# sbelharbi/sr-caco-2

Measured on AMD Instinct MI355X. Metric: train patches/sec, SwinIR x8 64->512 1ch, higher is better.
Workload: dtype f32 (fp16x2 split-MFMA, f32 accumulate)

## Files before the change

sr-caco-2_amd/csrc/gemm_tnb.hip:

```cpp
#include <stdlib.h>
#include "common.h"
#include "kernels.h"

typedef __bf16 bf16x8 __attribute__((ext_vector_type(8)));
typedef __bf16 bf16x2 __attribute__((ext_vector_type(2)));
typedef float f32x2 __attribute__((ext_vector_type(2)));
typedef unsigned u32x4 __attribute__((ext_vector_type(4)));

namespace {

constexpr int TKB = 32;

__device__ const float k_tnb_zero_row[256] = {0.f};

__device__ __forceinline__ f32x16 mfma_bf(u32x4 a, u32x4 b, f32x16 c) {
  return __builtin_amdgcn_mfma_f32_32x32x16_bf16(__builtin_bit_cast(bf16x8, a),
                                                 __builtin_bit_cast(bf16x8, b), c, 0, 0, 0);
}

typedef _Float16 f16x8 __attribute__((ext_vector_type(8)));
typedef _Float16 tn_f16x2 __attribute__((ext_vector_type(2)));
__device__ __forceinline__ f32x16 mfma_h(u32x4 a, u32x4 b, f32x16 c) {
  return __builtin_amdgcn_mfma_f32_32x32x16_f16(__builtin_bit_cast(f16x8, a), __builtin_bit_cast(f16x8, b), c, 0, 0, 0);
}
__device__ __forceinline__ void split2_pair(float x0, float x1, unsigned& h, unsigned& l) {
  const tn_f16x2 hv = __builtin_convertvector(f32x2{x0, x1}, tn_f16x2);
  const float r0 = x0 - (float)hv.x, r1 = x1 - (float)hv.y;
  const tn_f16x2 lv = __builtin_convertvector(f32x2{r0, r1}, tn_f16x2);
  h = __builtin_bit_cast(unsigned, hv);
  l = __builtin_bit_cast(unsigned, lv);
}

template <int W>
__device__ __forceinline__ int unit_slot(int col, int u) {
  if (W == 2) {
    const int x = col ^ (col >> 4);
    return 4 * ((col & ~3) | (x & 3)) + (u ^ ((x >> 2) & 3));
  }
  return 4 * col + (u ^ ((col >> 2) & 3));
}

typedef float tnb_f32x3 __attribute__((ext_vector_type(3)));
typedef tnb_f32x3 __attribute__((aligned(4))) tnb_f32x3_u;
template <int W> struct ColVec;
template <> struct ColVec<1> {
  typedef float T;
  static __device__ __forceinline__ T ldg(const float* p) { return ldg_f(p); }
  static __device__ __forceinline__ T ldg(const float* base, unsigned off) {
    return *(sr_gptr_f)((const char*)base + off);
  }
  static __device__ __forceinline__ float at(T v, int) { return v; }
};
template <> struct ColVec<2> {
  typedef sr_f32x2 T;
  static __device__ __forceinline__ T ldg(const float* p) { return *(sr_gptr_f2)p; }
  static __device__ __forceinline__ T ldg(const float* base, unsigned off) {
    return *(sr_gptr_f2)((const char*)base + off);
  }
  static __device__ __forceinline__ float at(T v, int j) { return v[j]; }
};
template <> struct ColVec<3> {
  typedef tnb_f32x3 T;
  static __device__ __forceinline__ T ldg(const float* p) {
    return *(const __attribute__((address_space(1))) tnb_f32x3_u*)p;
  }
  static __device__ __forceinline__ T ldg(const float* base, unsigned off) {
    return *(const __attribute__((address_space(1))) tnb_f32x3_u*)((const char*)base + off);
  }
  static __device__ __forceinline__ float at(T v, int j) { return v[j]; }
};

template <int W>
__device__ __forceinline__ void tnb_body(const TnArgs& p, const int s, const int tile, const int tap,
                                         unsigned char* smem) {
  constexpr int BC = 64 * W;
  constexpr int PLANE = 2 * BC * 64;
  constexpr int BUF = 3 * PLANE;

  const int tid = threadIdx.x, lane = tid & 63;
  const int wave8 = __builtin_amdgcn_readfirstlane(tid >> 6);
  const bool producer = wave8 >= 4;
  const int wave = wave8 & 3;
  const int wi = wave >> 1, wj = wave & 1, r = lane & 31, h = lane >> 5;
  const int nbj = (p.NJ + p.j_tile - 1) / p.j_tile;
  const int bi = tile / nbj, bj = tile - bi * nbj;
  const int i0 = bi * p.i_tile, j0 = bj * p.j_tile;
  const int ivalid = min(p.i_tile, p.NI - i0), jvalid = min(p.j_tile, p.NJ - j0);
  const int m_begin = s * p.rows_per_slice;
  const int m_end = min(p.M, m_begin + p.rows_per_slice);
  const int dy = p.conv ? tap / 3 - 1 : 0, dx = p.conv ? tap % 3 - 1 : 0;
  const bool do_colsum = p.part_colsum && bj == 0 && tap == 0;

  struct Stage {
    typename ColVec<W>::T rv[2][8];
// ... 183 lines not shown
    load(m_begin + TKB, sg1);
    store(smem, sg0);
    load(m_begin + 2 * TKB, sg0);
    __syncthreads();
    for (int c = 0; c < nch; c += 2) {
      store(smem + BUF, sg1);
      load(m_begin + (c + 3) * TKB, sg1);
      __syncthreads();
      store(smem, sg0);
      load(m_begin + (c + 4) * TKB, sg0);
      __syncthreads();
    }
  } else {
    __syncthreads();
    for (int c = 0; c < nch; ++c) {
      const unsigned char* cur = smem + (c & 1) * BUF;
#pragma unroll
      for (int ks = 0; ks < 2; ++ks) {
        u32x4 fa[W][3];
#pragma unroll
        for (int i = 0; i < W; ++i)
#pragma unroll
          for (int pl = 0; pl < 3; ++pl) fa[i][pl] = *(const u32x4*)(cur + pl * PLANE + a_off[i][ks]);
#pragma unroll
        for (int j = 0; j < W; ++j) {
          u32x4 fb0 = *(const u32x4*)(cur + b_off[j][ks]);
          u32x4 fb1 = *(const u32x4*)(cur + PLANE + b_off[j][ks]);
          u32x4 fb2 = *(const u32x4*)(cur + 2 * PLANE + b_off[j][ks]);
#pragma unroll
          for (int i = 0; i < W; ++i) acc[i][j] = mfma_bf(fa[i][1], fb1, acc[i][j]);
#pragma unroll
          for (int i = 0; i < W; ++i) acc[i][j] = mfma_bf(fa[i][0], fb2, acc[i][j]);
#pragma unroll
          for (int i = 0; i < W; ++i) acc[i][j] = mfma_bf(fa[i][2], fb0, acc[i][j]);
#pragma unroll
          for (int i = 0; i < W; ++i) acc[i][j] = mfma_bf(fa[i][0], fb1, acc[i][j]);
#pragma unroll
          for (int i = 0; i < W; ++i) acc[i][j] = mfma_bf(fa[i][1], fb0, acc[i][j]);
#pragma unroll
          for (int i = 0; i < W; ++i) acc[i][j] = mfma_bf(fa[i][0], fb0, acc[i][j]);
        }
      }
      __syncthreads();
    }

  float* out = p.part + ((long)(s * (p.conv ? 9 : 1) + tap) * p.NI) * p.NJ;
#pragma unroll
  for (int i = 0; i < W; ++i)
#pragma unroll
    for (int j = 0; j < W; ++j) {
      const int col = (wj * W + j) * 32 + r;
      if (col >= jvalid) continue;
#pragma unroll
      for (int q = 0; q < 16; ++q) {
        const int row = (wi * W + i) * 32 + mfma_row(q, lane);
        if (row < ivalid) {
          const int io = i0 + row;
          out[(long)(p.ps ? (io % ps_f) * 4 + io / ps_f : io) * p.NJ + j0 + col] = acc[i][j][q];
        }
      }
    }
  }

  if (do_colsum) {
    float* red = (float*)smem;
    if (producer && !isB) {
#pragma unroll
      for (int j = 0; j < W; ++j) red[hh * BC + W * lane + j] = cs[j];
    }
    __syncthreads();
    if (tid < ivalid) {
      const int io = i0 + tid;
      p.part_colsum[(long)s * p.NI + (p.ps ? (io % ps_f) * 4 + io / ps_f : io)] = red[tid] + red[BC + tid];
    }
  }
}

template <int W, int BM = -1, bool AR = false, bool NR = false, bool CONV = false>
__device__ __forceinline__ void tnb_body_h(const TnArgs& p, const int s, const int tile, unsigned char* smem, const int tap = 0) {
  const int bmode = BM >= 0 ? BM : p.b_mode;
  const bool arow = BM >= 0 ? AR : (p.a_rowscale != nullptr);
  constexpr int BC = 64 * W, HC = 32 * W;
  constexpr int PLANE = 2 * BC * 64;
  constexpr int BUF = 3 * PLANE;
  constexpr int CTRL = 2 * PLANE;
  constexpr int SINV = 2 * PLANE + 4096;

  const int tid = threadIdx.x, lane = tid & 63;
  const int wave8 = __builtin_amdgcn_readfirstlane(tid >> 6);
  const bool producer = wave8 >= 4;
  const int wave = wave8 & 3;
  const int wi = wave >> 1, wj = wave & 1, r = lane & 31, h = lane >> 5;
  const int nbj = (p.NJ + p.j_tile - 1) / p.j_tile;
  const int bi = tile / nbj, bj = tile - bi * nbj;
  const int i0 = bi * p.i_tile, j0 = bj * p.j_tile;
  const int ivalid = min(p.i_tile, p.NI - i0), jvalid = min(p.j_tile, p.NJ - j0);
  const int m_begin = s * p.rows_per_slice;
  const int m_end = min(p.M, m_begin + p.rows_per_slice);
  const bool do_colsum = p.part_colsum && bj == 0 && tap == 0;
  const int cdy = CONV ? tap / 3 - 1 : 0, cdx = CONV ? tap % 3 - 1 : 0;

  struct Stage {
    typename ColVec<W>::T rv[2][8];
    float scale;
    float2 stats;
    int trow;
  };
  Stage sg0, sg1;
  const bool isB = wave & 1;
  const int ch = wave >> 1;
  const int lt = lane & 31, th = lane >> 5;
  const int opvalid = isB ? jvalid : ivalid;
  const int gcol = HC * ch + W * lt;
  const int colq = max(min(gcol, opvalid - W), 0);
  const int dsh = gcol - colq;
  const bool ragged = NR ? false : opvalid % W != 0;
  const float* const opP = isB ? p.B + j0 : p.A + i0;
  const long opLd = isB ? p.ldb : p.lda;
  const unsigned colb = (unsigned)((16L * th * opLd + colq) * 4);
  float cs[W], sc[W];
#pragma unroll
  for (int j = 0; j < W; ++j) { cs[j] = 0.f; sc[j] = 0x1p126f; }

  auto bcast_i = [&](int v, int k) __attribute__((always_inline)) -> int {
    const int lo = __builtin_amdgcn_readlane(v, k), hi = __builtin_amdgcn_readlane(v, 16 + k);
    return th ? hi : lo;
  };
  const unsigned ld4 = (unsigned)opLd * 4u, colb0 = (unsigned)colq * 4u;
  auto load_c = [&](int mc, Stage& sg) __attribute__((always_inline)) {
    const int gm = mc + (lane & 31);
    bool ok = gm < m_end;
    int srow = gm;
    const int x = gm % p.Wd, tq = gm / p.Wd;
    const int y = tq % p.H, bq = tq / p.H;
    const int yy = y + (isB ? cdy : 0), xx = x + (isB ? cdx : 0);
    ok = ok && yy >= 0 && yy < p.H && xx >= 0 && xx < p.Wd;
    srow = (bq * p.H + yy) * p.Wd + xx;
    sg.trow = ok ? srow : -1;
#pragma unroll
    for (int t = 0; t < 16; ++t) {
      const int row = max(bcast_i(sg.trow, t), 0);
      sg.rv[t >> 3][t & 7] = ColVec<W>::ldg(opP, (unsigned)row * ld4 + colb0);
    }
  };
  auto load = [&](int mc, Stage& sg) __attribute__((always_inline)) {
    const int tokl = mc + (lane & 31);
    const bool interior = mc + TKB <= m_end;
    const bool tin = interior || tokl < m_end;
    if (!isB) sg.scale = ldg_f((arow && tin) ? p.a_rowscale + tokl / p.a_rowscale_rows : k_sr_neutral + 1);
    else sg.stats = ldg_f2((bmode == 1 && tin) ? p.ln_stats + 2 * (long)tokl : k_sr_neutral);
    const float* q = opP + (long)mc * opLd;
    if (interior) {
#pragma unroll
      for (int t = 0; t < 16; ++t) {
        sg.rv[t >> 3][t & 7] = ColVec<W>::ldg(q, colb);
        q += opLd;
      }
    } else {
#pragma unroll
      for (int t = 0; t < 16; ++t) {
        const bool ok = mc + 16 * th + t < m_end;
        sg.rv[t >> 3][t & 7] = ColVec<W>::ldg(ok ? (const float*)((const char*)q + colb) : k_tnb_zero_row);
        q += opLd;
      }
    }
  };
  auto load_i = [&](int mc, Stage& sg) __attribute__((always_inline)) {
// ... 175 lines not shown
      store(smem, sg0);
      load(m_begin + 2 * TKB, sg0);
      __syncthreads();
    }
    for (; c < nch; c += 2) {
      store(smem + BUF, sg1);
      load(m_begin + (c + 3) * TKB, sg1);
      __syncthreads();
      store(smem, sg0);
      load(m_begin + (c + 4) * TKB, sg0);
      __syncthreads();
    }
    if (th == 0) {
#pragma unroll
      for (int j = 0; j < W; ++j) ((float*)(smem + SINV))[(isB ? BC : 0) + gcol + j] = 1.0f / sc[j];
    }
    __syncthreads();
  } else {
    __syncthreads();
    for (int c = 0; c < nch; ++c) {
      const unsigned char* cur = smem + (c & 1) * BUF;
      const float* ctrl = (const float*)(cur + CTRL);
      const u32x4 fl = *(const u32x4*)(ctrl + 2 * BC);
      if (__builtin_amdgcn_readfirstlane(fl.x | fl.y | fl.z | fl.w)) {
        float fb[W];
#pragma unroll
        for (int j = 0; j < W; ++j) fb[j] = ctrl[BC + (wj * W + j) * 32 + r];
#pragma unroll
        for (int i = 0; i < W; ++i)
#pragma unroll
          for (int q = 0; q < 16; ++q) {
            const float fa = ctrl[(wi * W + i) * 32 + mfma_row(q, lane)];
#pragma unroll
            for (int j = 0; j < W; ++j) acc[i][j][q] *= fa * fb[j];
          }
      }
#pragma unroll
      for (int ks = 0; ks < 2; ++ks) {
        u32x4 fa[W][2];
#pragma unroll
        for (int i = 0; i < W; ++i)
#pragma unroll
          for (int pl = 0; pl < 2; ++pl) fa[i][pl] = *(const u32x4*)(cur + pl * PLANE + a_off[i][ks]);
#pragma unroll
        for (int j = 0; j < W; ++j) {
          const u32x4 bh = *(const u32x4*)(cur + b_off[j][ks]);
          const u32x4 bl = *(const u32x4*)(cur + PLANE + b_off[j][ks]);
#pragma unroll
          for (int i = 0; i < W; ++i) acc[i][j] = mfma_h(fa[i][1], bh, acc[i][j]);
#pragma unroll
          for (int i = 0; i < W; ++i) acc[i][j] = mfma_h(fa[i][0], bl, acc[i][j]);
#pragma unroll
          for (int i = 0; i < W; ++i) acc[i][j] = mfma_h(fa[i][0], bh, acc[i][j]);
        }
      }
      __syncthreads();
    }
    __syncthreads();
    const float* sinv = (const float*)(smem + SINV);
    float* out = p.part + ((long)(s * (CONV ? 9 : 1) + tap) * p.NI) * p.NJ;
#pragma unroll
    for (int i = 0; i < W; ++i)
#pragma unroll
      for (int j = 0; j < W; ++j) {
        const int col = (wj * W + j) * 32 + r;
        if (col >= jvalid) continue;
        const float ib = sinv[BC + col];
#pragma unroll
        for (int q = 0; q < 16; ++q) {
          const int row = (wi * W + i) * 32 + mfma_row(q, lane);
          if (row < ivalid) out[(long)(i0 + row) * p.NJ + j0 + col] = acc[i][j][q] * (sinv[row] * ib);
        }
      }
  }

  if (do_colsum) {
    float* red = (float*)smem;
    if (producer && !isB) {
#pragma unroll
      for (int j = 0; j < W; ++j) red[th * BC + gcol + j] = cs[j];
    }
    __syncthreads();
    if (tid < ivalid) p.part_colsum[(long)s * p.NI + i0 + tid] = red[tid] + red[BC + tid];
  }
}

constexpr int TK9 = 16;
__device__ __forceinline__ int unit_slot9(int col, int u) { return 2 * col + (u ^ ((col >> 3) & 1)); }
constexpr int T9_OPS = 6;
constexpr int T9_PLANE = T9_OPS * 64 * 32;
constexpr int T9_CTRL = 2 * T9_PLANE;
constexpr int T9_BUF = 2 * T9_PLANE + 2048;
constexpr int T9_SINV = 2 * T9_BUF;
constexpr int T9_LDS = 2 * T9_BUF + 2048;
constexpr int T9_THREADS = 14 * 64;

template <int H2, int DBG = 0>
__device__ __forceinline__ void tnb9_consume(const TnArgs& p, const int s, const int i0, const int j0, const int nch,
                                             unsigned char* smem, const int wi, const int wj, const int lane) {
  constexpr int NU = H2 ? 4 : 5;
  constexpr int DY0 = H2 ? 1 : 0;
  const int r = lane & 31, h = lane >> 5;
  f32x16 acc[NU];
#pragma unroll
  for (int u = 0; u < NU; ++u)
#pragma unroll
    for (int q = 0; q < 16; ++q) acc[u][q] = 0.f;
  int a_off[3], b_off[2];
#pragma unroll
  for (int d = 0; d < 3; ++d) a_off[d] = unit_slot9(d * 64 + wi * 32 + r, h) * 16;
#pragma unroll
  for (int d = 0; d < 2; ++d) b_off[d] = unit_slot9((3 + DY0 + d) * 64 + wj * 32 + r, h) * 16;
  __syncthreads();
  long long ts0 = 0, ts1 = 0;
  if (DBG == 3) ts0 = (long long)wall_clock64();
  for (int c = 0; c < nch; ++c) {
    const unsigned char* cur = smem + (c & 1) * T9_BUF;
    const float* ctrl = (const float*)(cur + T9_CTRL);
    const u32x4 f0 = *(const u32x4*)(ctrl + T9_OPS * 64);
    const sr_u32x2 f1 = *(const sr_u32x2*)(ctrl + T9_OPS * 64 + 4);
    if (__builtin_amdgcn_readfirstlane(f0.x | f0.y | f0.z | f0.w | f1.x | f1.y)) {
      const unsigned fl[6] = {f0.x, f0.y, f0.z, f0.w, f1.x, f1.y};
#pragma unroll
      for (int u = 0; u < NU; ++u) {
        constexpr int T0 = 5 * H2;
        const int t = T0 + u, dyi = t / 3, dxi = t - 3 * dyi;
        if (fl[dxi] | fl[3 + dyi]) {
          const float fb = fl[3 + dyi] ? ctrl[(3 + dyi) * 64 + wj * 32 + r] : 1.f;
#pragma unroll
          for (int q = 0; q < 16; ++q) acc[u][q] *= (fl[dxi] ? ctrl[dxi * 64 + wi * 32 + mfma_row(q, lane)] : 1.f) * fb;
        }
      }
    }
    u32x4 ah[3], al[3], bh[2], bl[2];
    const u32x4 dummy = u32x4{(unsigned)lane, 0x3c003c00u, 0x3c003c00u, (unsigned)c};
#pragma unroll
    for (int d = 0; d < 2; ++d) {
      bh[d] = (DBG >= 6) ? dummy : *(const u32x4*)(cur + b_off[d]);
      bl[d] = (DBG >= 6) ? dummy : *(const u32x4*)(cur + T9_PLANE + b_off[d]);
    }
#pragma unroll
    for (int dx = 0; dx < 3; ++dx) {
      ah[dx] = (DBG >= 6) ? dummy : *(const u32x4*)(cur + a_off[dx]);
      al[dx] = (DBG >= 6) ? dummy : *(const u32x4*)(cur + T9_PLANE + a_off[dx]);
    }
    if (DBG != 1) {
#pragma unroll
      for (int term = 0; term < 3; ++term) {
#pragma unroll
        for (int u = 0; u < NU; ++u) {
          const int t = 5 * H2 + u, dyi = t / 3, dxi = t - 3 * dyi;
          if (DBG == 10) {
            acc[u] = mfma_bf(term == 0 ? al[dxi] : ah[dxi], term == 1 ? bl[dyi - DY0] : bh[dyi - DY0], acc[u]);
          } else if (term == 0) acc[u] = mfma_h(al[dxi], bh[dyi - DY0], acc[u]);
          else if (term == 1) acc[u] = mfma_h(ah[dxi], bl[dyi - DY0], acc[u]);
          else acc[u] = mfma_h(ah[dxi], bh[dyi - DY0], acc[u]);
        }
      }
    }
    if (DBG != 8 && DBG != 10) __syncthreads();
  }
  if (DBG == 3) ts1 = (long long)wall_clock64();
  if (DBG != 9) __syncthreads();
  const float* sinv = (const float*)(smem + T9_SINV);
  const int col = wj * 32 + r;
  const int ps_f = p.NI >> 2;
// ... 402 lines not shown
      __syncthreads();
    }
    if (half == 0) ((float*)(smem + S9_SINV))[(isB ? 64 : 0) + lane] = 1.0f / sc;
    mxs[sw * 64 + lane] = mxrun;
    if (colsum && !isB) ((float*)(smem + S9_CS))[half * 64 + lane] = cs;
    __syncthreads();
    if (!pass) {
      aux[64 + sw * 64 + lane] = mxrun;
      const float mcol = fmaxf(mxrun, mxs[(sw ^ 1) * 64 + lane]);
      const float top = mcol * sc;
      const bool over = __any(top > 60000.f), under = __any(mcol > 0.f && top < 0.125f);
      if ((over || under) && lane == 0) *(volatile int*)(smem + S9_RETRY) = 1;
      if (lane == 0) ((int*)aux)[1 + sw] = (over ? 1 : 0) | (under ? 2 : 0);
    }
    __syncthreads();
    if (!pass && sw == 0 && lane == 0) *(int*)aux = *(volatile const int*)(smem + S9_RETRY);
  }
  if (colsum) {
    __syncthreads();
    if (sw == 0 && lane_ok) {
      const float* c2 = (const float*)(smem + S9_CS);
      const int io = i0 + lane;
      p.part_colsum[(long)s * p.NI + (p.ps ? (io % ps_f) * 4 + io / ps_f : io)] = c2[lane] + c2[64 + lane];
    }
  }
}

template <int DBG = 0, int PASS = 0>
__global__ void __launch_bounds__(S9_THREADS) k_tnb9s(TnArgs p, int tiles, int xcd) {
  extern __shared__ __attribute__((aligned(16))) unsigned char smem[];
  const int L = xcd ? sr_xcd_block(blockIdx.x, gridDim.x) : (int)blockIdx.x;
  tnb_body9s<DBG>(p, L / tiles, L % tiles, tiles, PASS, smem);
}

template <int W>
__global__ void __launch_bounds__(512, 1) k_tnb(TnArgs p, int tiles, int xcd) {
  extern __shared__ __attribute__((aligned(16))) unsigned char smem[];
  if (!p.conv) { tnb_body<W>(p, blockIdx.x, blockIdx.y, 0, smem); return; }
  const int L = xcd ? sr_xcd_block(blockIdx.x, gridDim.x) : (int)blockIdx.x;
  const int tap = L % 9, t2 = L / 9;
  tnb_body<W>(p, t2 / tiles, t2 % tiles, tap, smem);
}

template <int W>
__global__ void __launch_bounds__(512, 1) k_tnb_hc(TnArgs p, int tiles, int xcd) {
  extern __shared__ __attribute__((aligned(16))) unsigned char smem[];
  const int L = xcd ? sr_xcd_block(blockIdx.x, gridDim.x) : (int)blockIdx.x;
  const int tap = L % 9, t2 = L / 9;
  const bool even = p.NI % W == 0 && p.NJ % W == 0 && p.i_tile % W == 0 && p.j_tile % W == 0;
  if (even) tnb_body_h<W, 0, false, true, true>(p, t2 / tiles, t2 % tiles, smem, tap);
  else tnb_body_h<W, 0, false, false, true>(p, t2 / tiles, t2 % tiles, smem, tap);
}

constexpr int TNB_GROUP_MAX = 24;
struct TnbGroup {
  TnArgs p[TNB_GROUP_MAX];
  int tile_start[TNB_GROUP_MAX + 1];
  int n, S, xcd;
};
__device__ __forceinline__ void tnb_group_block(const TnbGroup& g, int& slice, int& t) {
  const int tiles = g.tile_start[g.n];
  if (g.xcd) {
    const int L = sr_xcd_block(blockIdx.x, gridDim.x);
    t = L % tiles;
    slice = L / tiles;
  } else {
    slice = blockIdx.x % g.S;
    t = blockIdx.x / g.S;
  }
}
template <int W>
__global__ void __launch_bounds__(512, 1) k_tnb_grouped(TnbGroup g) {
  extern __shared__ __attribute__((aligned(16))) unsigned char smem[];
  int slice, t;
  tnb_group_block(g, slice, t);
  TnArgs p = g.p[0];
  int t0 = 0;
#pragma unroll
  for (int i = 1; i < TNB_GROUP_MAX; ++i)
    if (i < g.n && t >= g.tile_start[i]) { p = g.p[i]; t0 = g.tile_start[i]; }
  tnb_body<W>(p, slice, t - t0, 0, smem);
}

template <int W>
__global__ void __launch_bounds__(512, 1) k_tnb_grouped_h(TnbGroup g) {
  extern __shared__ __attribute__((aligned(16))) unsigned char smem[];
  int slice, t;
  tnb_group_block(g, slice, t);
  TnArgs p = g.p[0];
  int t0 = 0;
#pragma unroll
  for (int i = 1; i < TNB_GROUP_MAX; ++i)
    if (i < g.n && t >= g.tile_start[i]) { p = g.p[i]; t0 = g.tile_start[i]; }
  const bool even = p.NI % W == 0 && p.NJ % W == 0 && p.i_tile % W == 0 && p.j_tile % W == 0;
  if (even && p.b_mode == 1 && !p.a_rowscale) tnb_body_h<W, 1, false, true>(p, slice, t - t0, smem);
  else if (even && p.b_mode == 0 && p.a_rowscale) tnb_body_h<W, 0, true, true>(p, slice, t - t0, smem);
  else if (even && p.b_mode == 2 && p.a_rowscale) tnb_body_h<W, 2, true, true>(p, slice, t - t0, smem);
  else tnb_body_h<W>(p, slice, t - t0, smem);
}

constexpr int TNB_BATCH_MAX = 40;
struct TnbConvBatch {
  TnArgs base;
  const float* A[TNB_BATCH_MAX];
  const float* B[TNB_BATCH_MAX];
  long part_stride, colsum_stride;
  int n, tiles, xcd;
};
template <int W>
__global__ void __launch_bounds__(512, 1) k_tnb_conv_batched(TnbConvBatch g) {
  extern __shared__ __attribute__((aligned(16))) unsigned char smem[];
  const int L = g.xcd ? sr_xcd_block(blockIdx.x, gridDim.x) : (int)blockIdx.x;
  const int tap = L % 9;
  int rr = L / 9;
  const int tile = rr % g.tiles; rr /= g.tiles;
  const int sl = rr % g.base.S, k = rr / g.base.S;
  TnArgs p = g.base;
  p.A = g.A[k];
  p.B = g.B[k];
  p.part = g.base.part + (long)k * g.part_stride;
  p.part_colsum = g.base.part_colsum ? g.base.part_colsum + (long)k * g.colsum_stride : nullptr;
  tnb_body<W>(p, sl, tile, tap, smem);
}

__global__ void __launch_bounds__(T9_THREADS) k_tnb9_conv_batched(TnbConvBatch g) {
  extern __shared__ __attribute__((aligned(16))) unsigned char smem[];
  const int L = g.xcd ? sr_xcd_block(blockIdx.x, gridDim.x) : (int)blockIdx.x;
  int rr = L;
  const int tile = rr % g.tiles; rr /= g.tiles;
  const int sl = rr % g.base.S, k = rr / g.base.S;
  TnArgs p = g.base;
  p.A = g.A[k];
  p.B = g.B[k];
  p.part = g.base.part + (long)k * g.part_stride;
  p.part_colsum = g.base.part_colsum ? g.base.part_colsum + (long)k * g.colsum_stride : nullptr;
  tnb_body9<0>(p, sl, tile, smem);
}

template <int PASS>
__global__ void __launch_bounds__(S9_THREADS) k_tnb9s_conv_batched(TnbConvBatch g) {
  extern __shared__ __attribute__((aligned(16))) unsigned char smem[];
  auto one = [&](int L) __attribute__((always_inline)) {
    int rr = L;
    const int tile = rr % g.tiles; rr /= g.tiles;
    const int sl = rr % g.base.S, k = rr / g.base.S;
    TnArgs p = g.base;
    p.A = g.A[k];
    p.B = g.B[k];
    p.part = g.base.part + (long)k * g.part_stride;
    p.part_colsum = g.base.part_colsum ? g.base.part_colsum + (long)k * g.colsum_stride : nullptr;
    p.aux = g.base.aux + (long)k * g.base.S * g.tiles * S9_AUX;
    tnb_body9s<0>(p, sl, tile, g.tiles, PASS, smem);
  };
  one(g.xcd ? sr_xcd_block(blockIdx.x, gridDim.x) : (int)blockIdx.x);
}

int pick_tile(int n, int* w) {
  if (n % 180 == 0) { *w = 3; return 180; }
  if (n <= 64) { *w = 1; return 64; }
  if (n <= 128 || n % 128 == 0) { *w = 2; return 128; }
  *w = 3; return 192;
}

int pick_w(int NI, int NJ, int* tile) {
  int wi, wj;
  const int ti = pick_tile(NI, &wi), tj = pick_tile(NJ, &wj);
  const int w = wi < wj ? wi : wj;
  *tile = wi == wj ? ti : (w == 3 ? 192 : 64 * w);
  if (wi == wj && ti != tj) *tile = 64 * w;
  return w;
}

enum TnbForm {
  TNB_PLAIN,
  TNB_HC,
  TNB_NINE,
  TNB_STRIP9,
};

TnbForm tnb_form(int conv, int NI, int NJ, const TnArgs* p = nullptr) {
#ifdef SR_TN_T9S_OFF
  constexpr int strip = 0;
#else
  static const int strip = [] { const char* e = sr_getenv("SRHIP_TN_T9S"); return !(e && e[0] == '0'); }();
#endif
  static const int ragged = [] { const char* e = sr_getenv("SRHIP_TN_T9S_RAGGED"); return e ? atoi(e) : 1; }();
  static const int f16c3 = [] { const char* e = sr_getenv("SRHIP_TN_F16X2_CONV3"); return e ? atoi(e) : 1; }();
  if (!conv || (p && (p->a_rowscale || p->b_mode != 0))) return TNB_PLAIN;
  int tile;
  const int w = pick_w(NI, NJ, &tile);
  const bool nine = w == 1 && NI % 64 == 0 && NJ % 64 == 0;
  if (strip && (nine || (ragged && NI >= 64 && NJ >= 64)) &&
      (!p || (p->Wd % 64 == 0 && p->S >= p->Wd / 64 && (!p->ps || NI % 64 == 0) &&
              (long)p->batch * p->H * (p->Wd / 64) >= 4L * p->S)))
    return TNB_STRIP9;
  if (nine) return TNB_NINE;
  if (w >= 2 && f16c3 &&
      (!p || (!p->ps && (long)p->M * p->lda < (1L << 30) && (long)p->batch * p->H * p->Wd * p->ldb < (1L << 30))))
    return TNB_HC;
  return TNB_PLAIN;
}
TnbForm tnb_form(const TnArgs& p) { return tnb_form(p.conv, p.NI, p.NJ, &p); }

long tnb_plan_blocks(int conv, int NI, int NJ, int* w, bool* nine) {
  int tile;
  *w = pick_w(NI, NJ, &tile);
  const TnbForm f = tnb_form(conv, NI, NJ);
  *nine = f == TNB_NINE || f == TNB_STRIP9;
  if (f == TNB_STRIP9) tile = 64;
  return (long)sr_cdiv(NI, tile) * sr_cdiv(NJ, tile) * (conv && !*nine ? 9 : 1);
}

template <typename K>
int reserve_lds(K kern, int bytes, const char* name) {
  hipError_t e = hipFuncSetAttribute((const void*)kern, hipFuncAttributeMaxDynamicSharedMemorySize, bytes);
  if (e != hipSuccess) return sr_fail(-5, "%s: cannot reserve %d B of LDS: %s", name, bytes, hipGetErrorString(e));
  return 0;
}

constexpr int lds_bytes(int w) { return 2 * 3 * 2 * 64 * w * 64; }
constexpr long TNB_W1_SLOTS = 3 * 256;

}

int sr_gemm_tnb_grouped(TnArgs* probs, int n, hipStream_t st) {
  SR_REQUIRE(n >= 1 && n <= TNB_GROUP_MAX, "gemm_tn_grouped_bx3: 1..%d problems (got %d)", TNB_GROUP_MAX, n);
  static_assert(sizeof(TnbGroup) <= 4096, "kernel arguments");
  TnbGroup g;
  memset(&g, 0, sizeof(g));
  g.n = n;
  int w = 1, tiles = 0;
  for (int k = 0; k < n; ++k) {
    TnArgs& p = probs[k];
    SR_REQUIRE(p.M == probs[0].M && p.S == probs[0].S && !p.conv,
               "gemm_tn_grouped_bx3: problems must share M and S");
    SR_REQUIRE(p.NI % 4 == 0 && p.NJ % 4 == 0 && p.lda % 4 == 0 && p.ldb % 4 == 0,
               "gemm_tn_grouped_bx3: NI, NJ, lda, ldb must be multiples of 4");
    int a, b;
    p.i_tile = pick_tile(p.NI, &a);
    p.j_tile = pick_tile(p.NJ, &b);
    if (a > w) w = a;
    if (b > w) w = b;
    const int rps = sr_cdiv(p.M, p.S);
    p.rows_per_slice = (rps + TKB - 1) / TKB * TKB;
    g.tile_start[k] = tiles;
    tiles += sr_cdiv(p.NI, p.i_tile) * sr_cdiv(p.NJ, p.j_tile);
    g.p[k] = p;
  }
  g.tile_start[n] = tiles;
  g.S = probs[0].S;
  static const int gxcd = [] { const char* e = sr_getenv("SRHIP_TN_GROUP_XCD"); return e ? atoi(e) : 1; }();
  g.xcd = gxcd;
  dim3 grid(probs[0].S * tiles, 1, 1);
  static bool attr[4] = {false, false, false, false};
#define SR_TNB_G(W_)                                                                      \
  if (w == W_) {                                                                          \
    if (!attr[W_]) {                                                                      \
      if (int rc = reserve_lds(k_tnb_grouped<W_>, lds_bytes(W_), "k_tnb_grouped")) return rc; \
      attr[W_] = true;                                                                    \
    }                                                                                     \
    hipLaunchKernelGGL((k_tnb_grouped<W_>), grid, dim3(512), lds_bytes(W_), st, g);       \
  }
  if (w == 3) {
    static bool attr_h = false;
    if (!attr_h) {
      if (int rc = reserve_lds(k_tnb_grouped_h<3>, lds_bytes(3), "k_tnb_grouped_h")) return rc;
      attr_h = true;
    }
    hipLaunchKernelGGL((k_tnb_grouped_h<3>), grid, dim3(512), lds_bytes(3), st, g);
  }
  SR_TNB_G(1) SR_TNB_G(2)
#undef SR_TNB_G
  SR_LAUNCH_CHECK("k_tnb_grouped");
  return 0;
}

int sr_gemm_tnb(TnArgs& p, hipStream_t st) {
  SR_REQUIRE(p.M > 0 && p.S > 0, "gemm_tn_bx3: empty problem");
  SR_REQUIRE(p.NI % 4 == 0 && p.NJ % 4 == 0 && p.lda % 4 == 0 && p.ldb % 4 == 0,
             "gemm_tn_bx3: NI, NJ, lda, ldb must be multiples of 4");
  int tile;
  const int w = pick_w(p.NI, p.NJ, &tile);
  p.i_tile = p.j_tile = tile;
  SR_REQUIRE(!p.ps || (p.conv && p.NI % 4 == 0 && (p.NI / 4) % w == 0 && p.NI % p.i_tile == 0),
             "conv3x3_wgrad + PixelShuffle(2): Cout/4 = %d must be a multiple of %d (columns per lane), Cout of the tile", p.NI / 4, w);
  const int rps = sr_cdiv(p.M, p.S);
  p.rows_per_slice = (rps + TKB - 1) / TKB * TKB;
  int tiles = sr_cdiv(p.NI, p.i_tile) * sr_cdiv(p.NJ, p.j_tile);
  dim3 grid(p.S, tiles, 1);
  if (p.conv) grid = dim3(p.S * tiles * 9, 1, 1);
  static const int xcd = [] { const char* e = sr_getenv("SRHIP_TN_XCD"); return !(e && e[0] == '0'); }();
  const TnbForm form = tnb_form(p);
  if (form == TNB_STRIP9) {
    p.i_tile = p.j_tile = 64;
    tiles = sr_cdiv(p.NI, 64) * sr_cdiv(p.NJ, 64);
    p.aux = p.part + (long)p.S * 9 * p.NI * p.NJ;
    static bool attr9s = false;
    if (!attr9s) {
      if (int rc = reserve_lds(k_tnb9s<0, 0>, S9_LDS, "k_tnb9s")) return rc;
      if (int rc = reserve_lds(k_tnb9s<0, 1>, S9_LDS, "k_tnb9s")) return rc;
      attr9s = true;
    }
#ifdef SRHIP_EXPERIMENTS
    {
      const char* e = sr_getenv("SRHIP_TN_DBG");
      const int dbg = e ? atoi(e) : 0;
#define SR_T9DBG(D_) if (dbg == D_) { reserve_lds(k_tnb9s<D_>, S9_LDS, "k_tnb9s"); hipLaunchKernelGGL(k_tnb9s<D_>, dim3(p.S * tiles), dim3(S9_THREADS), S9_LDS, st, p, tiles, xcd); return 0; }
      SR_T9DBG(1) SR_T9DBG(2) SR_T9DBG(6) SR_T9DBG(7)
#undef SR_T9DBG
    }
#endif
    hipLaunchKernelGGL((k_tnb9s<0, 0>), dim3(p.S * tiles), dim3(S9_THREADS), S9_LDS, st, p, tiles, xcd);
    hipLaunchKernelGGL((k_tnb9s<0, 1>), dim3(p.S * tiles), dim3(S9_THREADS), S9_LDS, st, p, tiles, xcd);
    SR_LAUNCH_CHECK("k_tnb9s");
    return 0;
  }
  if (form == TNB_NINE) {
    static bool attr9 = false;
    if (!attr9) {
      if (int rc = reserve_lds(k_tnb9<0>, T9_LDS, "k_tnb9")) return rc;
      attr9 = true;
    }
#ifdef SRHIP_EXPERIMENTS
    {
      const char* e = sr_getenv("SRHIP_TN_DBG");
      const int dbg = e ? atoi(e) : 0;
#define SR_T9DBG(D_) if (dbg == D_) { reserve_lds(k_tnb9<D_>, T9_LDS, "k_tnb9"); hipLaunchKernelGGL(k_tnb9<D_>, dim3(p.S * tiles), dim3(T9_THREADS), T9_LDS, st, p, tiles, xcd); return 0; }
      SR_T9DBG(1) SR_T9DBG(2) SR_T9DBG(6) SR_T9DBG(7) SR_T9DBG(3) SR_T9DBG(8) SR_T9DBG(9) SR_T9DBG(10) SR_T9DBG(4) SR_T9DBG(5)
#undef SR_T9DBG
    }
#endif
    hipLaunchKernelGGL(k_tnb9<0>, dim3(p.S * tiles), dim3(T9_THREADS), T9_LDS, st, p, tiles, xcd);
    SR_LAUNCH_CHECK("k_tnb9");
    return 0;
  }
  if (form == TNB_HC) {
    static bool attr_hc[4] = {false, false, false, false};
#define SR_TNB_HC(W_)                                                                       \
    if (w == W_) {                                                                          \
      if (!attr_hc[W_]) {                                                                   \
        if (int rc = reserve_lds(k_tnb_hc<W_>, lds_bytes(W_), "k_tnb_hc")) return rc;       \
        attr_hc[W_] = true;                                                                 \
      }                                                                                     \
      hipLaunchKernelGGL((k_tnb_hc<W_>), grid, dim3(512), lds_bytes(W_), st, p, tiles, xcd); \
    }
    SR_TNB_HC(2) SR_TNB_HC(3)
#undef SR_TNB_HC
    SR_LAUNCH_CHECK("k_tnb_hc");
    return 0;
  }
  static bool attr[4] = {false, false, false, false};
#define SR_TNB(W_)                                                                        \
  if (w == W_) {                                                                          \
    if (!attr[W_]) {                                                                      \
      if (int rc = reserve_lds(k_tnb<W_>, lds_bytes(W_), "k_tnb")) return rc;             \
      attr[W_] = true;                                                                    \
    }                                                                                     \
    hipLaunchKernelGGL((k_tnb<W_>), grid, dim3(512), lds_bytes(W_), st, p, tiles, xcd);   \
  }
  SR_TNB(1) SR_TNB(2) SR_TNB(3)
#undef SR_TNB
  SR_LAUNCH_CHECK("k_tnb");
  return 0;
}

int sr_conv_wgrad_batched_plan(int n, int M, int NI, int NJ, int* S, long* part_floats_per_item) {
  int w;
  bool t9;
  const long tiles = tnb_plan_blocks(1, NI, NJ, &w, &t9) * n;
  const long slots = w == 1 && !t9 ? TNB_W1_SLOTS : 256;
  long best = 1;
  double best_eff = 0.0;
  for (long s = 1; s <= 64; ++s) {
    if (s > 1 && M / s < 1024) break;
    const long blocks = tiles * s;
    const double eff = (double)blocks / (double)(((blocks + slots - 1) / slots) * slots);
    if (eff > best_eff + 0.02) { best_eff = eff; best = s; }
  }
  *S = (int)best;
  *part_floats_per_item = best * 9 * (long)NI * NJ + (t9 ? best * (tiles / n) * S9_AUX : 0);
  return 0;
}

int sr_conv_wgrad_batched_tnb(const TnArgs& base, const float* const* A, const float* const* B, int n,
                              long part_stride, long colsum_stride, hipStream_t st) {
  SR_REQUIRE(n >= 1 && n <= TNB_BATCH_MAX, "conv3x3_wgrad_batched: 1..%d problems (got %d)", TNB_BATCH_MAX, n);
  SR_REQUIRE(base.conv && base.M > 0 && base.S > 0, "conv3x3_wgrad_batched: conv problems only");
  SR_REQUIRE(base.NI % 4 == 0 && base.NJ % 4 == 0 && base.lda % 4 == 0 && base.ldb % 4 == 0,
             "conv3x3_wgrad_batched: Cout, Cin and the pixel pitches must be multiples of 4");
  TnbConvBatch g;
  memset(&g, 0, sizeof(g));
  g.base = base;
  int tile;
  const int w = pick_w(base.NI, base.NJ, &tile);
  g.base.i_tile = g.base.j_tile = tile;
  const int rps = sr_cdiv(base.M, base.S);
  g.base.rows_per_slice = (rps + TKB - 1) / TKB * TKB;
  g.n = n;
  g.tiles = sr_cdiv(base.NI, tile) * sr_cdiv(base.NJ, tile);
  g.part_stride = part_stride;
  g.colsum_stride = colsum_stride;
  for (int k = 0; k < n; ++k) { g.A[k] = A[k]; g.B[k] = B[k]; }
  static const int xcd = [] { const char* e = sr_getenv("SRHIP_TN_XCD"); return !(e && e[0] == '0'); }();
  g.xcd = xcd;
  const TnbForm form = tnb_form(g.base);
  if (form == TNB_STRIP9) {
    g.base.i_tile = g.base.j_tile = 64;
    g.tiles = sr_cdiv(base.NI, 64) * sr_cdiv(base.NJ, 64);
    g.base.aux = base.part + (long)n * part_stride;
    static bool attr9s = false;
    if (!attr9s) {
      if (int rc = reserve_lds(k_tnb9s_conv_batched<0>, S9_LDS, "k_tnb9s_conv_batched")) return rc;
      if (int rc = reserve_lds(k_tnb9s_conv_batched<1>, S9_LDS, "k_tnb9s_conv_batched")) return rc;
      attr9s = true;
    }
    hipLaunchKernelGGL(k_tnb9s_conv_batched<0>, dim3(base.S * g.tiles * n), dim3(S9_THREADS), S9_LDS, st, g);
    hipLaunchKernelGGL(k_tnb9s_conv_batched<1>, dim3(base.S * g.tiles * n), dim3(S9_THREADS), S9_LDS, st, g);
    SR_LAUNCH_CHECK("k_tnb9s_conv_batched");
    return 0;
  }
  if (form == TNB_NINE) {
    static bool attr9 = false;
    if (!attr9) {
      if (int rc = reserve_lds(k_tnb9_conv_batched, T9_LDS, "k_tnb9_conv_batched")) return rc;
      attr9 = true;
    }
    hipLaunchKernelGGL(k_tnb9_conv_batched, dim3(base.S * g.tiles * n), dim3(T9_THREADS), T9_LDS, st, g);
// ... 35 lines not shown
```

Baseline: 726.0.

## Add 16-wave grouped fp16x2 TN GEMM kernel with split consumer quadrants

Adds a 1024-thread variant of the grouped W=3 TN weight-gradient GEMM. Eight producer waves each stage one operand's column quarter, and eight consumer waves split each 3x3 MFMA quadrant into 5- and 4-tile halves, so more waves are resident to hide load and MFMA latency. The LDS buffer layout is reduced to double buffering, and the old kernel now gets smaller LDS sizing for the h and hc paths. The older 512-thread kernel stays as a fallback for forms the new path does not handle. The risks are more synchronisation across 16 waves and register pressure.

After: 726.7 (median of 2 runs). No clear change (+0.1%).

```diff
diff --git a/sr-caco-2_amd/csrc/gemm_tnb.hip b/sr-caco-2_amd/csrc/gemm_tnb.hip
--- a/sr-caco-2_amd/csrc/gemm_tnb.hip
+++ b/sr-caco-2_amd/csrc/gemm_tnb.hip
@@ -1,4 +1,5 @@
 #include <stdlib.h>
+#include <type_traits>
 #include "common.h"
 #include "kernels.h"
 
@@ -10,6 +11,8 @@
 namespace {
 
 constexpr int TKB = 32;
+constexpr int lds_bytes(int w) { return 2 * 3 * 2 * 64 * w * 64; }
+constexpr int lds_bytes_h(int w) { return 2 * (2 * 2 * 64 * w * 64 + 8192); }
 
 __device__ const float k_tnb_zero_row[256] = {0.f};
 
@@ -359,7 +362,7 @@
   const bool arow = BM >= 0 ? AR : (p.a_rowscale != nullptr);
   constexpr int BC = 64 * W, HC = 32 * W;
   constexpr int PLANE = 2 * BC * 64;
-  constexpr int BUF = 3 * PLANE;
+  constexpr int BUF = lds_bytes_h(W) / 2;
   constexpr int CTRL = 2 * PLANE;
   constexpr int SINV = 2 * PLANE + 4096;
 
@@ -701,6 +704,340 @@
     }
     __syncthreads();
     if (tid < ivalid) p.part_colsum[(long)s * p.NI + i0 + tid] = red[tid] + red[BC + tid];
+  }
+}
+
+constexpr int H16_THREADS = 1024;
+template <int W> struct H16 {
+  static constexpr int BC = 64 * W;
+  static constexpr int PLANE = 2 * BC * 64;
+  static constexpr int CTRL = 2 * PLANE;
+  static constexpr int BUF = 2 * PLANE + 2048;
+  static constexpr int SINV = 2 * BUF;
+  static constexpr int LDS = 2 * BUF + 2048;
+  static_assert(2 * BC * 4 + 32 <= 2048 && 4 * BC * 4 <= BUF, "control block / column-sum scratch");
+  static_assert(LDS <= 160 * 1024, "LDS of one CU");
+};
+
+template <int K>
+__device__ __forceinline__ float row_bcast(float v) {
+  return __builtin_bit_cast(float, __builtin_amdgcn_update_dpp(0, __builtin_bit_cast(int, v), 0x150 + K, 0xf, 0xf, false));
+}
+__device__ __forceinline__ void row_bcast8(float v, float (&o)[8]) {
+  o[0] = row_bcast<0>(v); o[1] = row_bcast<1>(v); o[2] = row_bcast<2>(v); o[3] = row_bcast<3>(v);
+  o[4] = row_bcast<4>(v); o[5] = row_bcast<5>(v); o[6] = row_bcast<6>(v); o[7] = row_bcast<7>(v);
+}
+
+template <int W, int BM = -1, bool AR = false, bool NR = false, int DBG = 0>
+__device__ __forceinline__ void tnb_body_h16(const TnArgs& p, const int s, const int tile, unsigned char* smem) {
+  static_assert(W == 3, "the 5 / 4 cut of a quadrant is the one of 3 x 3 MFMA tiles");
+  const int bmode = BM >= 0 ? BM : p.b_mode;
+  const bool arow = BM >= 0 ? AR : (p.a_rowscale != nullptr);
+  constexpr int BC = H16<W>::BC, QC = 16 * W;
+  constexpr int PLANE = H16<W>::PLANE, BUF = H16<W>::BUF, CTRL = H16<W>::CTRL, SINV = H16<W>::SINV;
+
+  const int tid = threadIdx.x, lane = tid & 63;
+  const int wave16 = __builtin_amdgcn_readfirstlane(tid >> 6);
+  const bool producer = wave16 >= 8;
+  const int nbj = (p.NJ + p.j_tile - 1) / p.j_tile;
+  const int bi = tile / nbj, bj = tile - bi * nbj;
+  const int i0 = bi * p.i_tile, j0 = bj * p.j_tile;
+  const int ivalid = min(p.i_tile, p.NI - i0), jvalid = min(p.j_tile, p.NJ - j0);
+  const int m_begin = s * p.rows_per_slice;
+  const int m_end = min(p.M, m_begin + p.rows_per_slice);
+  const bool do_colsum = p.part_colsum && bj == 0;
+  const int nch = ((m_end - m_begin + 2 * TKB - 1) / (2 * TKB)) * 2;
+
+  if (producer) {
+    struct Stage {
+      typename ColVec<W>::T rv[8];
+      float scale;
+      float2 stats;
+    };
+    const int sw = wave16 & 7;
+    auto stage = [&](auto operand) __attribute__((always_inline)) {
+    constexpr bool isB = decltype(operand)::value;
+    Stage sg0, sg1;
+    const int cq = sw >> 1;
+    const int lt = lane & 15, tq = lane >> 4;
+    const int opvalid = isB ? jvalid : ivalid;
+    const int gcol = QC * cq + W * lt;
+    const int colq = max(min(gcol, opvalid - W), 0);
+    const int dsh = gcol - colq;
+    const bool ragged = NR ? false : opvalid % W != 0;
+    const float* const opP = isB ? p.B + j0 : p.A + i0;
+    const long opLd = isB ? p.ldb : p.lda;
+    const unsigned colb = (unsigned)((8L * tq * opLd + colq) * 4);
+    const int tsub = 8 * tq + (lane & 7);
+    float cs[W], sc[W];
+#pragma unroll
+    for (int j = 0; j < W; ++j) { cs[j] = 0.f; sc[j] = 0x1p126f; }
+
+    auto load = [&](int mc, Stage& sg) __attribute__((always_inline)) {
+      if (DBG == 2) return;
+      const int tokl = mc + tsub;
+      const bool interior = mc + TKB <= m_end;
+      const bool tin = interior || tokl < m_end;
+      if (!isB) sg.scale = ldg_f((arow && tin) ? p.a_rowscale + tokl / p.a_rowscale_rows : k_sr_neutral + 1);
+      else sg.stats = ldg_f2((bmode == 1 && tin) ? p.ln_stats + 2 * (long)tokl : k_sr_neutral);
+      const float* q = opP + (long)mc * opLd;
+      if (interior) {
+#pragma unroll
+        for (int t = 0; t < 8; ++t) {
+          sg.rv[t] = ColVec<W>::ldg(q, colb);
+          q += opLd;
+        }
+      } else {
+#pragma unroll
+        for (int t = 0; t < 8; ++t) {
+          const bool ok = mc + 8 * tq + t < m_end;
+          sg.rv[t] = ColVec<W>::ldg(ok ? (const float*)((const char*)q + colb) : k_tnb_zero_row);
+          q += opLd;
+        }
+      }
+    };
+    auto load_i = [&](int mc, Stage& sg) __attribute__((always_inline)) {
+      if (DBG == 2) return;
+      const int tokl = mc + tsub;
+      if (BM < 0 || AR) sg.scale = ldg_f((!isB && arow) ? p.a_rowscale + tokl / p.a_rowscale_rows : k_sr_neutral + 1);
+      if (BM < 0 || BM == 1) sg.stats = ldg_f2((isB && bmode == 1) ? p.ln_stats + 2 * (long)tokl : k_sr_neutral);
+      const float* q = opP + (long)mc * opLd;
+#pragma unroll
+      for (int t = 0; t < 8; ++t) {
+        sg.rv[t] = ColVec<W>::ldg(q, colb);
+        q += opLd;
+      }
+    };
+    auto store = [&](unsigned char* buf, const Stage& sg) {
+      if (DBG == 2) return;
+      sr_f32x2 x[4][W];
+      if (!ragged) {
+#pragma unroll
+        for (int t = 0; t < 4; ++t)
+#pragma unroll
+          for (int j = 0; j < W; ++j)
+            x[t][j] = sr_f32x2{ColVec<W>::at(sg.rv[2 * t], j), ColVec<W>::at(sg.rv[2 * t + 1], j)};
+      } else {
+#pragma unroll
+        for (int t = 0; t < 4; ++t)
+#pragma unroll
+          for (int j = 0; j < W; ++j) {
+            float e0 = ColVec<W>::at(sg.rv[2 * t], W - 1), e1 = ColVec<W>::at(sg.rv[2 * t + 1], W - 1);
+#pragma unroll
+            for (int d = W - 2; d >= 0; --d)
+              if (j + d < W && dsh == d) {
+                e0 = ColVec<W>::at(sg.rv[2 * t], j + d);
+                e1 = ColVec<W>::at(sg.rv[2 * t + 1], j + d);
+              }
+            x[t][j] = sr_f32x2{e0, e1};
+          }
+      }
+      if (!isB) {
+        if (arow) {
+          float k[8];
+          row_bcast8(sg.scale, k);
+#pragma unroll
+          for (int t = 0; t < 4; ++t)
+#pragma unroll
+            for (int j = 0; j < W; ++j) { x[t][j].x *= k[2 * t]; x[t][j].y *= k[2 * t + 1]; }
+        }
+        if (do_colsum) {
+#pragma unroll
+          for (int t = 0; t < 4; ++t)
+#pragma unroll
+            for (int j = 0; j < W; ++j) cs[j] += x[t][j].x + x[t][j].y;
+        }
+      } else if (bmode == 1) {
+        float mu[8], rs[8];
+        row_bcast8(sg.stats.x, mu);
+        row_bcast8(sg.stats.y, rs);
+#pragma unroll
+        for (int t = 0; t < 4; ++t)
+#pragma unroll
+          for (int j = 0; j < W; ++j) {
+            x[t][j].x = (x[t][j].x - mu[2 * t]) * rs[2 * t];
+            x[t][j].y = (x[t][j].y - mu[2 * t + 1]) * rs[2 * t + 1];
+          }
+      } else if (bmode == 2) {
+#pragma unroll
+        for (int t = 0; t < 4; ++t)
+#pragma unroll
+          for (int j = 0; j < W; ++j) x[t][j] = gelu_fast2(x[t][j]);
+      }
+      float f[W];
+      bool chg = false;
+#pragma unroll
+      for (int j = 0; j < W; ++j) {
+        float mx = 0.f;
+#pragma unroll
+        for (int t = 0; t < 4; ++t) mx = fmaxf(mx, fmaxf(fabsf(x[t][j].x), fabsf(x[t][j].y)));
+        mx = fmaxf(mx, __shfl_xor(mx, 16));
+        mx = fmaxf(mx, __shfl_xor(mx, 32));
+        f[j] = 1.f;
+        if (mx * sc[j] > 60000.f) {
+          const float ns = exp2f(fminf(floorf(log2f(16384.f / mx)), 120.f));
+          f[j] = ns / sc[j];
+          sc[j] = ns;
+          chg = true;
+        }
+      }
+      const bool any = __any(chg);
+      float* ctrl = (float*)(buf + CTRL);
+      if (tq == 0) {
+#pragma unroll
+        for (int j = 0; j < W; ++j) ctrl[(isB ? BC : 0) + gcol + j] = f[j];
+      }
+      if (lane == 0) ((int*)(ctrl + 2 * BC))[sw] = any ? 1 : 0;
+#pragma unroll
+      for (int j = 0; j < W; ++j) {
+        unsigned qh[4], ql[4];
+#pragma unroll
+        for (int t = 0; t < 4; ++t) split2_pair(x[t][j].x * sc[j], x[t][j].y * sc[j], qh[t], ql[t]);
+        unsigned char* dst = buf + unit_slot<W>((isB ? BC : 0) + gcol + j, tq) * 16;
+        *(u32x4*)(dst) = u32x4{qh[0], qh[1], qh[2], qh[3]};
+        *(u32x4*)(dst + PLANE) = u32x4{ql[0], ql[1], ql[2], ql[3]};
+      }
+    };
+
+    __builtin_amdgcn_s_setprio(2);
+    const int n_int = (m_end - m_begin) / TKB;
+    int c = 0;
+    if (n_int >= 5) {
+      load_i(m_begin, sg0);
+      load_i(m_begin + TKB, sg1);
+      store(smem, sg0);
+      load_i(m_begin + 2 * TKB, sg0);
+      __syncthreads();
+      for (; c + 4 < n_int; c += 2) {
+        store(smem + BUF, sg1);
+        load_i(m_begin + (c + 3) * TKB, sg1);
+        __syncthreads();
+        store(smem, sg0);
+        load_i(m_begin + (c + 4) * TKB, sg0);
+        __syncthreads();
+      }
+    } else {
+      load(m_begin, sg0);
+      load(m_begin + TKB, sg1);
+      store(smem, sg0);
+      load(m_begin + 2 * TKB, sg0);
+      __syncthreads();
+    }
+    for (; c < nch; c += 2) {
+      store(smem + BUF, sg1);
+      load(m_begin + (c + 3) * TKB, sg1);
+      __syncthreads();
+      store(smem, sg0);
+      load(m_begin + (c + 4) * TKB, sg0);
+      __syncthreads();
+    }
+    if (tq == 0) {
+#pragma unroll
+      for (int j = 0; j < W; ++j) ((float*)(smem + SINV))[(isB ? BC : 0) + gcol + j] = 1.0f / sc[j];
+    }
+    __syncthreads();
+    if (do_colsum) {
+      float* red = (float*)smem;
+      if (!isB) {
+#pragma unroll
+        for (int j = 0; j < W; ++j) red[tq * BC + gcol + j] = cs[j];
+      }
+    }
+    };
+    if (((sw >> 2) ^ sw) & 1) stage(std::integral_constant<bool, true>());
+    else stage(std::integral_constant<bool, false>());
+  } else {
+    const int qd = wave16 & 3, wi = qd >> 1, wj = qd & 1, r = lane & 31, h = lane >> 5;
+    auto consume = [&](auto half) __attribute__((always_inline)) {
+      constexpr int HF = decltype(half)::value;
+      constexpr int NT = HF ? 4 : 5;
+      constexpr int ka[5] = {0, 0, 0, 1, 1}, kb[5] = {0, 1, 2, 0, 1};
+      constexpr int ti[2] = {HF ? 2 : 0, 1}, tj[3] = {HF ? 2 : 0, 1, HF ? 0 : 2};
+      f32x16 acc[NT];
+#pragma unroll
+      for (int k = 0; k < NT; ++k)
+#pragma unroll
+        for (int q = 0; q < 16; ++q) acc[k][q] = 0.f;
+      int a_off[2][2], b_off[3][2];
+#pragma unroll
+      for (int i = 0; i < 2; ++i)
+#pragma unroll
+        for (int ks = 0; ks < 2; ++ks) a_off[i][ks] = unit_slot<W>((wi * W + ti[i]) * 32 + r, 2 * ks + h) * 16;
+#pragma unroll
+      for (int j = 0; j < 3; ++j)
+#pragma unroll
+        for (int ks = 0; ks < 2; ++ks) b_off[j][ks] = unit_slot<W>(BC + (wj * W + tj[j]) * 32 + r, 2 * ks + h) * 16;
+
+      __syncthreads();
+      for (int c = 0; c < nch; ++c) {
+        const unsigned char* cur = smem + (c & 1) * BUF;
+        const float* ctrl = (const float*)(cur + CTRL);
+        if (DBG != 2) {
+          const u32x4 f0 = *(const u32x4*)(ctrl + 2 * BC), f1 = *(const u32x4*)(ctrl + 2 * BC + 4);
+          if (__builtin_amdgcn_readfirstlane(f0.x | f0.y | f0.z | f0.w | f1.x | f1.y | f1.z | f1.w)) {
+            float fb[3];
+#pragma unroll
+            for (int j = 0; j < 3; ++j) fb[j] = ctrl[BC + (wj * W + tj[j]) * 32 + r];
+#pragma unroll
+            for (int i = 0; i < 2; ++i)
+#pragma unroll
+              for (int q = 0; q < 16; ++q) {
+                const float fa = ctrl[(wi * W + ti[i]) * 32 + mfma_row(q, lane)];
+#pragma unroll
+                for (int k = 0; k < NT; ++k)
+                  if (ka[k] == i) acc[k][q] *= fa * fb[kb[k]];
+              }
+          }
+        }
+        if (DBG != 1) {
+#pragma unroll
+          for (int ks = 0; ks < 2; ++ks) {
+            u32x4 fa[2][2];
+#pragma unroll
+            for (int i = 0; i < 2; ++i)
+#pragma unroll
+              for (int pl = 0; pl < 2; ++pl) fa[i][pl] = *(const u32x4*)(cur + pl * PLANE + a_off[i][ks]);
+#pragma unroll
+            for (int j = 0; j < 3; ++j) {
+              const u32x4 bh = *(const u32x4*)(cur + b_off[j][ks]);
+              const u32x4 bl = *(const u32x4*)(cur + PLANE + b_off[j][ks]);
+#pragma unroll
+              for (int k = 0; k < NT; ++k)
+                if (kb[k] == j) acc[k] = mfma_h(fa[ka[k]][1], bh, acc[k]);
+#pragma unroll
+              for (int k = 0; k < NT; ++k)
+                if (kb[k] == j) acc[k] = mfma_h(fa[ka[k]][0], bl, acc[k]);
+#pragma unroll
+              for (int k = 0; k < NT; ++k)
+                if (kb[k] == j) acc[k] = mfma_h(fa[ka[k]][0], bh, acc[k]);
+            }
+          }
+        }
+        __syncthreads();
+      }
+      __syncthreads();
+      const float* sinv = (const float*)(smem + SINV);
+      float* out = p.part + ((long)s * p.NI) * p.NJ;
+#pragma unroll
+      for (int k = 0; k < NT; ++k) {
+        const int col = (wj * W + tj[kb[k]]) * 32 + r;
+        if (col >= jvalid) continue;
+        const float ib = sinv[BC + col];
+#pragma unroll
+        for (int q = 0; q < 16; ++q) {
+          const int row = (wi * W + ti[ka[k]]) * 32 + mfma_row(q, lane);
+          if (row < ivalid) out[(long)(i0 + row) * p.NJ + j0 + col] = acc[k][q] * (sinv[row] * ib);
+        }
+      }
+    };
+    if (wave16 >= 4) consume(std::integral_constant<int, 1>());
+    else consume(std::integral_constant<int, 0>());
+  }
+
+  if (do_colsum) {
+    const float* red = (const float*)smem;
+    __syncthreads();
+    if (tid < ivalid) p.part_colsum[(long)s * p.NI + i0 + tid] = (red[tid] + red[BC + tid]) + (red[2 * BC + tid] + red[3 * BC + tid]);
   }
 }
 
@@ -1269,6 +1606,31 @@
   tnb_body<W>(p, slice, t - t0, 0, smem);
 }
 
+__host__ __device__ __forceinline__ int h16_form(const TnArgs& p, int W) {
+  if (p.NI % W || p.NJ % W || p.i_tile % W || p.j_tile % W) return 0;
+  if (p.b_mode == 1 && !p.a_rowscale) return 1;
+  if (p.b_mode == 0) return p.a_rowscale ? 2 : 4;
+  if (p.b_mode == 2 && p.a_rowscale) return 3;
+  return 0;
+}
+
+template <int W, int DBG = 0>
+__global__ void __launch_bounds__(H16_THREADS) k_tnb_grouped_h16(TnbGroup g) {
+  extern __shared__ __attribute__((aligned(16))) unsigned char smem[];
+  int slice, t;
+  tnb_group_block(g, slice, t);
+  TnArgs p = g.p[0];
+  int t0 = 0;
+#pragma unroll
+  for (int i = 1; i < TNB_GROUP_MAX; ++i)
+    if (i < g.n && t >= g.tile_start[i]) { p = g.p[i]; t0 = g.tile_start[i]; }
+  const int form = h16_form(p, W);
+  if (form == 1) tnb_body_h16<W, 1, false, true, DBG>(p, slice, t - t0, smem);
+  else if (form == 2) tnb_body_h16<W, 0, true, true, DBG>(p, slice, t - t0, smem);
+  else if (form == 3) tnb_body_h16<W, 2, true, true, DBG>(p, slice, t - t0, smem);
+  else tnb_body_h16<W, 0, false, true, DBG>(p, slice, t - t0, smem);
+}
+
 template <int W>
 __global__ void __launch_bounds__(512, 1) k_tnb_grouped_h(TnbGroup g) {
   extern __shared__ __attribute__((aligned(16))) unsigned char smem[];
@@ -1279,11 +1641,7 @@
 #pragma unroll
   for (int i = 1; i < TNB_GROUP_MAX; ++i)
     if (i < g.n && t >= g.tile_start[i]) { p = g.p[i]; t0 = g.tile_start[i]; }
-  const bool even = p.NI % W == 0 && p.NJ % W == 0 && p.i_tile % W == 0 && p.j_tile % W == 0;
-  if (even && p.b_mode == 1 && !p.a_rowscale) tnb_body_h<W, 1, false, true>(p, slice, t - t0, smem);
-  else if (even && p.b_mode == 0 && p.a_rowscale) tnb_body_h<W, 0, true, true>(p, slice, t - t0, smem);
-  else if (even && p.b_mode == 2 && p.a_rowscale) tnb_body_h<W, 2, true, true>(p, slice, t - t0, smem);
-  else tnb_body_h<W>(p, slice, t - t0, smem);
+  tnb_body_h<W>(p, slice, t - t0, smem);
 }
 
 constexpr int TNB_BATCH_MAX = 40;
@@ -1405,7 +1763,6 @@
   return 0;
 }
 
-constexpr int lds_bytes(int w) { return 2 * 3 * 2 * 64 * w * 64; }
 constexpr long TNB_W1_SLOTS = 3 * 256;
 
 }
@@ -1449,12 +1806,29 @@
     hipLaunchKernelGGL((k_tnb_grouped<W_>), grid, dim3(512), lds_bytes(W_), st, g);       \
   }
   if (w == 3) {
+    bool forms = true;
+    for (int k = 0; k < n; ++k) forms = forms && h16_form(g.p[k], 3) != 0;
     static bool attr_h = false;
     if (!attr_h) {
-      if (int rc = reserve_lds(k_tnb_grouped_h<3>, lds_bytes(3), "k_tnb_grouped_h")) return rc;
+      if (int rc = reserve_lds(k_tnb_grouped_h16<3>, H16<3>::LDS, "k_tnb_grouped_h16")) return rc;
+      if (int rc = reserve_lds(k_tnb_grouped_h<3>, lds_bytes_h(3), "k_tnb_grouped_h")) return rc;
       attr_h = true;
     }
-    hipLaunchKernelGGL((k_tnb_grouped_h<3>), grid, dim3(512), lds_bytes(3), st, g);
+    if (!forms) {
+      hipLaunchKernelGGL((k_tnb_grouped_h<3>), grid, dim3(512), lds_bytes_h(3), st, g);
+      SR_LAUNCH_CHECK("k_tnb_grouped_h");
+      return 0;
+    }
+#ifdef SRHIP_EXPERIMENTS
+    {
+      const char* e = sr_getenv("SRHIP_TN_DBG");
+      const int dbg = e ? atoi(e) : 0;
+#define SR_H16DBG(D_) if (dbg == D_) { reserve_lds(k_tnb_grouped_h16<3, D_>, H16<3>::LDS, "k_tnb_grouped_h16"); hipLaunchKernelGGL((k_tnb_grouped_h16<3, D_>), grid, dim3(H16_THREADS), H16<3>::LDS, st, g); return 0; }
+      SR_H16DBG(1) SR_H16DBG(2)
+#undef SR_H16DBG
+    }
+#endif
+    hipLaunchKernelGGL((k_tnb_grouped_h16<3>), grid, dim3(H16_THREADS), H16<3>::LDS, st, g);
   }
   SR_TNB_G(1) SR_TNB_G(2)
 #undef SR_TNB_G
@@ -1526,10 +1900,10 @@
 #define SR_TNB_HC(W_)                                                                       \
     if (w == W_) {                                                                          \
       if (!attr_hc[W_]) {                                                                   \
-        if (int rc = reserve_lds(k_tnb_hc<W_>, lds_bytes(W_), "k_tnb_hc")) return rc;       \
+        if (int rc = reserve_lds(k_tnb_hc<W_>, lds_bytes_h(W_), "k_tnb_hc")) return rc;     \
         attr_hc[W_] = true;                                                                 \
       }                                                                                     \
-      hipLaunchKernelGGL((k_tnb_hc<W_>), grid, dim3(512), lds_bytes(W_), st, p, tiles, xcd); \
+      hipLaunchKernelGGL((k_tnb_hc<W_>), grid, dim3(512), lds_bytes_h(W_), st, p, tiles, xcd); \
     }
     SR_TNB_HC(2) SR_TNB_HC(3)
 #undef SR_TNB_HC
```
